# axruff/cuda-flow3d

Measured on AMD Instinct MI355X. Metric: Mvoxels/s full pyramid solve, higher is better.
Workload: dtype f32; 1 GPU; 512^3 synthetic translated-Gaussian float32 pair (BASELINE config 4), full coarse-to-fine pyramid (40 levels x 40 outer x 5 inner, alpha 7.5, median 5^3, Gaussian sigma 2), frames resident in HBM (value = device-resident rate); parallelism=1 GPU

## Files before the change

cuda-flow3d_amd/csrc/f3d_pair8_plan.h:

```cpp
#pragma once

#include <algorithm>
#include <cstdlib>
#include <vector>

#if !defined(__HIPCC__) && !defined(__host__)
#define __host__
#define __device__
#define F3D_PAIR8_PLAN_OWN_QUALIFIERS
#endif

constexpr int kPair8Lanes = 64;

#if defined(__HIP_DEVICE_COMPILE__)
#define PAIR8_UNIFORM(x) __builtin_amdgcn_readfirstlane(x)
#else
#define PAIR8_UNIFORM(x) (x)
#endif

inline int solver_chunk_limit(unsigned long long plane_bytes, int reach)
{
  if (plane_bytes == 0 || plane_bytes > 0x100000000ull || reach < 0) return 0;
  const long long planes = static_cast<long long>(0xffffffffull / plane_bytes) - 8;
  if (planes >= 1) return planes > 0x3fffffff ? 0x3fffffff : static_cast<int>(planes);
// ... 42 lines not shown
  const int n_a = tiles_a * PAIR8_UNIFORM(c.chunks_a), n_b = tiles_b * PAIR8_UNIFORM(c.chunks_b), n_c = tiles_c * PAIR8_UNIFORM(c.chunks_c);
  int cls;
  int item;
  if (xcd_remap) {
    const int per_a = (n_a + 7) / 8, per_b = (n_b + 7) / 8, per_c = (n_c + 7) / 8;
    const int xcd = wg % 8, s = wg / 8;
    cls = s < per_a ? 0 : (s < per_a + per_b ? 1 : 2);
    item = cls == 0 ? xcd * per_a + s : (cls == 1 ? xcd * per_b + (s - per_a) : xcd * per_c + (s - per_a - per_b));
  } else {
    cls = wg < n_a ? 0 : (wg < n_a + n_b ? 1 : 2);
    item = cls == 0 ? wg : (cls == 1 ? wg - n_a : wg - n_a - n_b);
  }
  if (item >= (cls == 0 ? n_a : (cls == 1 ? n_b : n_c))) return false;
  const int tiles = cls == 0 ? tiles_a : (cls == 1 ? tiles_b : tiles_c);
  const int zc = cls == 0 ? zc_a : (cls == 1 ? zc_b : zc_c);
  const int chunk = item / tiles;
  w.tile = item % tiles + (cls == 0 ? 0 : (cls == 1 ? tiles_a : tiles_a + tiles_b));
  w.z0 = m_lo + chunk * zc;
  w.z1 = w.z0 + zc + more < m_hi ? w.z0 + zc + more : m_hi;
  if (fold) {
    const int pair = w.tile / (2 * ntx - 1), k = w.tile % (2 * ntx - 1);
    w.folded = k == ntx - 1;
    w.tx = k < ntx ? k : k - ntx;
    w.ty = k < ntx ? 2 * pair : 2 * pair + 1;
  } else {
    w.folded = false;
    w.tx = w.tile % ntx;
    w.ty = w.tile / ntx;
  }
  return true;
}

__host__ __device__ constexpr int pair8_slot_halo_off(int ns, int nj) { return ns * nj * kPair8Lanes; }
__host__ __device__ constexpr int pair8_slot_floats(int ns, int nj)
{
  return pair8_slot_halo_off(ns, nj) + (ns * 2 * nj + kPair8Lanes - 1) / kPair8Lanes * 4 * kPair8Lanes;
}
struct Pair8XNeighbours {
  int left, right;
};
__host__ __device__ inline Pair8XNeighbours pair8_x_neighbours(int lane, int x0, int width)
{
  const int x = x0 + lane;
  Pair8XNeighbours n = {lane - 1, lane + 1};
  if (x == 0) n.left = n.right;
  if (x == width - 1) n.right = n.left;
  return n;
}
__host__ __device__ inline int pair8_x_neighbour_offset(int elem, int array, int row, int ns, int nj)
{
  const int halo = pair8_slot_halo_off(ns, nj) + (array * 2 * nj + row) * 4;
  if (elem < 0) return halo + 3;
  if (elem >= kPair8Lanes) return halo + nj * 4;
  return (array * nj + row) * kPair8Lanes + elem;
}

struct Pair8Plan {
  int zchunk;
  long cost;
  long wgs = 0;
  Pair8Cut cut = {};
};
inline Pair8Cut pair8_uniform_cut(int tiles, int planes, int zchunk)
{
  return Pair8Cut{0, 0, 0, tiles, (planes + zchunk - 1) / zchunk, zchunk, 0, 0, 0};
}
inline long pair8_per_round(long standard)
{
  const char* e = std::getenv("F3D_PAIR8_ROUND");
  const long v = e ? std::atol(e) : 0;
  return v > 0 ? v : standard;
}
inline int pair8_chunk_steps()
{
  static const int extra = std::getenv("F3D_PAIR8_CHUNK_STEPS") ? std::atoi(std::getenv("F3D_PAIR8_CHUNK_STEPS")) : 7;
  return extra;
}
inline Pair8Plan pair8_plan_two(int width, int rows, int planes, int ty, int zc_limit, long per_round, bool fold, bool two_class)
{
  const long tiles = pair8_tiles_per_chunk((width + kPair8Lanes - 1) / kPair8Lanes, (rows + ty - 1) / ty, fold);
  const int max_chunks = planes > 0 ? planes : 1;
  const int extra = pair8_chunk_steps();
  auto rounds = [&](long wgs) { return (wgs + per_round - 1) / per_round; };
  Pair8Plan p = {std::min(planes, zc_limit), -1};
  for (int nzc = 1; nzc <= max_chunks; ++nzc) {
    const int zc = (planes + nzc - 1) / nzc;
    if (zc > zc_limit) continue;
    const long wgs = tiles * ((planes + zc - 1) / zc);
    const long cost = rounds(wgs) * (zc + extra);
    if (p.cost < 0 || cost < p.cost) {
      p.cost = cost;
      p.zchunk = zc;
      p.wgs = wgs;
    }
  }
  if (p.cost < 0) {
    p.cost = static_cast<long>(rounds(tiles)) * (p.zchunk + extra);
    p.wgs = tiles;
  }
  if (p.zchunk < 1) p.zchunk = 1;
  p.cut = pair8_uniform_cut(static_cast<int>(tiles), planes, p.zchunk);
  if (!two_class || tiles <= per_round || planes < 1 || zc_limit < 1) return p;
  const int a0 = (planes + zc_limit - 1) / zc_limit;
  int zc_a_seen = 0;
  for (int na = a0; na <= a0 + 2 && na <= planes; ++na) {
    const int zc_a = (planes + na - 1) / na;
// ... 126 lines not shown
```

cuda-flow3d_amd/csrc/f3d_solve_pair8.h:

```cpp

enum { PAIR_SS = 0, PAIR_SP = 1, PAIR_PS = 2, PAIR_SSA = 3 };

struct PairArgs {
  const float* in[12];
  float* out[5];
  float hx, hy, hz, alpha;
  float eps_s, eps_d;
  int plain_division;
  int keep_below, keep_above;
  double r4[3], r2[3];
  float d4[3], d2[3];
  float w[3];
  float eps_s2, eps_d2;
  int fdivs_ok, sdivs_ok;
};

inline bool pair_weights_finite(float hx, float hy, float hz, float alpha)
{
  for (float h : {hx, hy, hz}) {
    const float w = alpha / (h * h);
    if (!(w - w == 0.f) || std::signbit(w)) return false;
  }
  return true;
}
// ... 138 lines not shown
    phi = w_phi;
    ksi = w_ksi;
  } else {
    phi = weight_ieee(a_phi);
    ksi = weight_ieee(a_ksi);
  }
}

__device__ __forceinline__ void weights_first_stage1(float (&q)[9], bool with_ksi, float fx, float fy, float fz, float ft, float du,
                                                     float dv_c, float dw, const SolveDivs& dv, float eps_s2, float eps_d2, float& phi,
                                                     float& ksi, bool counts, bool fast_weights)
{
  if (__builtin_expect(dv.ok, 1)) {
#pragma unroll
    for (int c = 0; c < 3; ++c) {
      q[3 * c + 0] = udiv(q[3 * c + 0], dv.x2);
      q[3 * c + 1] = udiv(q[3 * c + 1], dv.y2);
      q[3 * c + 2] = udiv(q[3 * c + 2], dv.z2);
    }
  } else {
#pragma unroll
    for (int c = 0; c < 3; ++c) {
      q[3 * c + 0] = q[3 * c + 0] / dv.x2.d;
      q[3 * c + 1] = q[3 * c + 1] / dv.y2.d;
      q[3 * c + 2] = q[3 * c + 2] / dv.z2.d;
    }
  }
  const float dux = q[0], duy = q[1], duz = q[2], dvx = q[3], dvy = q[4], dvz = q[5], dwx = q[6], dwy = q[7], dwz = q[8];
  const float a_phi = dux * dux + duy * duy + duz * duz + dvx * dvx + dvy * dvy + dvz * dvz + dwx * dwx + dwy * dwy + dwz * dwz + eps_s2;
  float s_phi, s_ksi = 1.f, a_ksi = 1.f, w_ksi = 0.f;
  const float w_phi = weight_fast(a_phi, s_phi);
  bool lane_ok = weight_fast_ok(a_phi, s_phi);
  if (with_ksi) {
    const float J11 = fx * fx, J22 = fy * fy, J33 = fz * fz;
    const float J12 = fx * fy, J13 = fx * fz, J23 = fy * fz;
    const float J14 = fx * ft, J24 = fy * ft, J34 = fz * ft, J44 = ft * ft;
    float s = (J11 * du + J12 * dv_c + J13 * dw + J14) * du + (J12 * du + J22 * dv_c + J23 * dw + J24) * dv_c +
              (J13 * du + J23 * dv_c + J33 * dw + J34) * dw + (J14 * du + J24 * dv_c + J34 * dw + J44);
    s = static_cast<float>(s > 0) * s;
    a_ksi = s + eps_d2;
    w_ksi = weight_fast(a_ksi, s_ksi);
    lane_ok = lane_ok && weight_fast_ok(a_ksi, s_ksi);
  }
  if (__builtin_expect(fast_weights && __builtin_amdgcn_ballot_w64(counts && !lane_ok) == 0, 1)) {
    phi = w_phi;
    ksi = w_ksi;
  } else {
    phi = weight_ieee(a_phi);
    ksi = with_ksi ? weight_ieee(a_ksi) : 0.f;
  }
}


template <int MODE, int TY, int ABL, bool FD, bool YM, bool TIGHT, bool FOLDS = false>
__device__ __forceinline__ void pair8_body(const PairArgs& a, const F3dGeo& g, const Pair8Cut& cut, int ntx, int nty, int xcd_remap)
{
  static_assert(!FOLDS || (!YM && !TIGHT && ABL == 0), "two row bands per tile: z-marching product builds only");
  static_assert(!(YM && FD), "the frame-derivative launchers march along z only");
  static_assert(!TIGHT || (YM && ABL == 0), "a tile without halo rows holds every row of the volume: thin volumes marched along y");
  constexpr bool PS = MODE == PAIR_PS;
  constexpr bool SSM = MODE == PAIR_SS || MODE == PAIR_SSA;
  static_assert((!PS && MODE != PAIR_SSA) || (FD && !YM && !TIGHT && ABL == 0), "k_wpair8: frame-derivative z-marching product builds only");
  constexpr int RH = TIGHT ? 0 : 1;
  const int RDIM = YM ? g.D : g.H;
  const int MDIM = YM ? g.H : g.D;
  const int m_lo = YM ? 0 : g.z_lo, m_hi = YM ? g.H : g.z_hi;
  constexpr int NA = FD ? 12 : 10;
  using L = Pair8Lds<TY, NA, FD, TIGHT, PS>;
  constexpr int NR = L::NR, NJ = L::NJ, NK = L::NK, NJP = L::NJP, NH = L::NH;
  static_assert(TY <= 32, "the column wave holds one halo voxel per lane: 2 x TY <= 64");
  __shared__ __attribute__((aligned(16))) float ring[L::kSlots][L::kSlotFloats];
  __shared__ __attribute__((aligned(16))) float cring[L::kCSlots][L::kCSlotFloats];
  constexpr int SB = FD ? 2 : 0;
  constexpr int NI = PS ? 4 : 3;
  constexpr int IW = kLanes + 2;
  constexpr int IS = (NR * IW + 63) / 64 * 64;
  __shared__ float imgx[2][PS ? NI : 1][PS ? IS : 1];
  __shared__ float img1[2][NI][PS ? 1 : NR][kLanes];
  __shared__ float hc1[2][NI][2][32];
  __shared__ float img3[(ABL & 64) ? 3 : 1][(ABL & 64) ? NR : 1][(ABL & 64) ? kLanes : 1];

  Pair8Wg wg;
  if (!pair8_decode(static_cast<int>(blockIdx.x), cut, ntx, nty, FOLDS, xcd_remap, m_lo, m_hi, (ABL & 64) ? 1 : 0, wg)) return;
  const int tx = wg.tx, ty = wg.ty;
  const bool folded = wg.folded;

  auto tile_body = [&](auto fold_c) __attribute__((always_inline)) {
  constexpr bool FOLD = decltype(fold_c)::value;
  int lane = threadIdx.x;
  const int r = __builtin_amdgcn_readfirstlane(static_cast<int>(threadIdx.y));
  const bool colw = r == NR;
  const bool loader = r == NR + 1;
  const int z0 = wg.z0, z1 = wg.z1;
  const int qs = z0 > 0 ? z0 - 1 : 0;
  const int qe = z1 < MDIM ? z1 : MDIM - 1;
  const int q_end = z1 < MDIM ? qe : qe + 1;
  const int p_last = qe + 1;
  const int x0 = tx * kLanes;
  const int y0 = ty * TY;
  const bool left_face = tx == 0;
  const bool right_face = x0 + kLanes >= g.W;
  const bool tile_at_x_face = __builtin_amdgcn_readfirstlane(static_cast<int>(left_face || right_face)) != 0;
  const bool col_at_x_face = __builtin_amdgcn_readfirstlane(static_cast<int>(left_face || right_face || x0 + kLanes == g.W - 1)) != 0;

  const int st_lo = (a.keep_below && z0 == m_lo) ? z0 - 1 : z0;
  const int st_hi = (a.keep_above && z1 == m_hi) ? z1 + 1 : z1;
  const int zb = qs > 0 ? qs - 1 : 0;
  const unsigned z_stride_b = static_cast<unsigned>(g.Hc) * static_cast<unsigned>(g.pitch) * 4u;
  const unsigned y_stride_b = static_cast<unsigned>(g.pitch) * 4u;
  const unsigned plane_b = YM ? y_stride_b : z_stride_b;
  const unsigned row_b = YM ? z_stride_b : y_stride_b;
  const size_t base_off = YM ? static_cast<size_t>(zb) * static_cast<size_t>(g.pitch) : f3d_row(g, 0, zb);

  if (loader) {
    __builtin_amdgcn_s_setprio(3);
    const float* base[NA];
#pragma unroll
    for (int i = 0; i < NA; ++i) base[i] = (PS && (i == 8 || i == 9)) ? nullptr : uniform_ptr(a.in[i] + base_off);
    const bool bandb = FOLD && (lane & 15) >= 8;
    const int seg = bandb ? (lane & 15) - 8 : (lane & 15);
    unsigned rowb[NK];
    bool rowv[NK];
#pragma unroll
    for (int k = 0; k < NK; ++k) {
      const int j = 4 * k + (lane >> 4);
      rowv[k] = j < NJ;
      const int yrow = f3d_clampi(f3d_mir(y0 + (bandb ? TY : 0) - 2 * RH + (rowv[k] ? j : 0), RDIM), 0, RDIM - 1);
      rowb[k] = static_cast<unsigned>(yrow) * row_b + static_cast<unsigned>(x0 + 4 * seg) * 4u;
    }
    const float* hptr[NH];
    bool hv[NH];
#pragma unroll
// ... 152 lines not shown
        static_cast<int>(static_cast<unsigned>(zz - zb) * plane_b + static_cast<unsigned>(yrow) * row_b)));
  };

  float seedv = static_cast<float>(lane) * 0.01f + 1.f;
  auto fake_raw = [&](PlaneRegs& p) __attribute__((always_inline)) {
    p.f0 = opaque(seedv); p.f1 = opaque(seedv); p.u = opaque(seedv); p.v = opaque(seedv); p.w = opaque(seedv);
    p.su = opaque(seedv); p.dv = opaque(seedv); p.dw = opaque(seedv); p.phi = opaque(seedv); p.ksi = opaque(seedv);
    p.fz = opaque(seedv); p.ft = opaque(seedv);
  };
  auto row_raw = [&](PlaneRegs& p, const float* slot, int j, bool with_ksi, const float* cs = nullptr) __attribute__((always_inline)) {
    if (ABL & 8) return fake_raw(p);
    const float* d = slot + j * kLanes + lane;
    constexpr int st = NJP * kLanes;
    if (!FD) {
      p.f0 = d[F0 * st];
      p.f1 = d[F1 * st];
    }
    p.u = d[(U - SB) * st]; p.v = d[(V - SB) * st]; p.w = d[(Wf - SB) * st];
    p.su = d[(DU - SB) * st]; p.dv = d[(DV - SB) * st]; p.dw = d[(DW - SB) * st]; p.phi = d[(PHI - SB) * st];
    if (!FD && with_ksi) p.ksi = d[9 * st];
    if (FD && !with_ksi) p.f0 = p.f1 = 0.f;
    if (FD && with_ksi) {
      const float* c = cs + (j - 1) * kLanes + lane;
      constexpr int ct = L::NRC * kLanes;
      p.f0 = c[0 * ct]; p.f1 = c[1 * ct]; p.ksi = c[2 * ct]; p.fz = c[3 * ct]; p.ft = c[4 * ct];
    }
  };
  auto halo_raw = [&](PlaneRegs& p, const float* slot, int s, int j, int e, bool with_ksi, const float* cs = nullptr) __attribute__((always_inline)) {
    if (ABL & 8) return fake_raw(p);
    const float* d = slot + L::kHaloOff + (s * NJ + j) * 4 + e;
    constexpr int st = 2 * NJ * 4;
    if (!FD) {
      p.f0 = d[F0 * st];
      p.f1 = d[F1 * st];
    }
    p.u = d[(U - SB) * st]; p.v = d[(V - SB) * st]; p.w = d[(Wf - SB) * st];
    p.su = d[(DU - SB) * st]; p.dv = d[(DV - SB) * st]; p.dw = d[(DW - SB) * st]; p.phi = d[(PHI - SB) * st];
    if (!FD && with_ksi) p.ksi = d[9 * st];
    if (FD && !with_ksi) p.f0 = p.f1 = 0.f;
    if (FD && with_ksi) {
      const float* c = cs + L::kCHaloOff + (s * TY + (j - 2)) * 4 + e;
      constexpr int ct = 2 * TY * 4;
      p.f0 = c[0 * ct]; p.f1 = c[1 * ct]; p.ksi = c[2 * ct]; p.fz = c[3 * ct]; p.ft = c[4 * ct];
    }
  };

  S3 hM = {0.f, 0.f, 0.f}, hC = {0.f, 0.f, 0.f};
  float hC_dv = 0.f, hC_dw = 0.f;
  Carry kC = {};
  Carry kC2 = {};
  CarryP pC = {};

  Face6 nYm = {}, nYp = {}, nX = {};
  S3 nDy = {0.f, 0.f, 0.f}, nXr = {0.f, 0.f, 0.f};
  Face6 nIn = {};
  S3 nInr = {0.f, 0.f, 0.f};
  auto fetch_neighbours = [&](auto colw_c, const float* S) __attribute__((always_inline)) {
    constexpr bool CW = decltype(colw_c)::value;
    PlaneRegs T0, T1, T2;
    if constexpr (CW) {
      PlaneRegs T;
      const float* d = S + jc * kLanes + (side ? (FOLD ? 32 : kLanes - 1) : 0);
      constexpr int st = NJP * kLanes;
      if (ABL & 8) {
        fake_raw(T);
      } else {
        if (!FD) {
          T.f0 = d[F0 * st];
          T.f1 = d[F1 * st];
        } else {
          T.f0 = T.f1 = 0.f;
        }
        T.u = d[(U - SB) * st]; T.v = d[(V - SB) * st]; T.w = d[(Wf - SB) * st];
        T.su = d[(DU - SB) * st]; T.dv = d[(DV - SB) * st]; T.dw = d[(DW - SB) * st]; T.phi = d[(PHI - SB) * st];
      }
      nInr = {T.u, T.v, T.w};
      plane_finish(T);
      nIn = plane_face(T);
    }
    if constexpr (CW) {
      halo_raw(T0, S, side, jc_m, e_near, false);
      halo_raw(T1, S, side, jc_p, e_near, false);
      halo_raw(T2, S, side, jc, e_far, false);
    } else {
      row_raw(T0, S, jr_m, false);
      row_raw(T1, S, jr_p, false);
      halo_raw(T2, S, side, jr, e_near, false);
    }
    if (MODE == PAIR_SP) {
      nDy = {T1.u - T0.u, T1.v - T0.v, T1.w - T0.w};
      nXr = {T2.u, T2.v, T2.w};
    }
    plane_finish(T0);
    plane_finish(T1);
    plane_finish(T2);
    nYm = plane_face(T0);
    nYp = plane_face(T1);
    nX = plane_face(T2);
  };

  auto step = [&](auto colw_c, auto slot_c, PlaneRegs& M, PlaneRegs& C, PlaneRegs& P, int q) __attribute__((always_inline)) {
    constexpr bool CW = decltype(colw_c)::value;
    constexpr int SLOT = decltype(slot_c)::value;
    if constexpr (TY > 8 || TIGHT) lane = fresh_lane();
    const int band = FOLD ? lane >> 5 : 0;
    if (!(ABL & 8)) __syncthreads();
    if (ABL & 4) return;
    const float* Sp = &ring[SLOT][0];
    const float* Cp = &cring[FD ? ((q + 1 - qs) & 1) : 0][0];
    const bool do1 = q <= qe;
    const int b = q & 1;

    float r_du = 0.f, r_dv = 0.f, r_dw = 0.f;
    Carry kN;
    CarryP pN;
    {
      Face6 xm, xp;
      const Face6 ym = nYm, yp = nYp;
      S3 rxm = {}, rxp = {};
      int vx, vy;
      if constexpr (CW) {
        halo_raw(P, Sp, side, jc, e_near, true, Cp);
        plane_finish(P);
        const S3 router = nXr;
        const Face6 outer = nX;
        const S3 rinner = nInr;
        const Face6 inner = nIn;
#pragma unroll
        for (int i = 0; i < kNL; ++i) {
          xm.v[i] = !FOLD && side ? inner.v[i] : outer.v[i];
          xp.v[i] = !FOLD && side ? outer.v[i] : inner.v[i];
        }
        rxm = !FOLD && side ? rinner : router;
        rxp = !FOLD && side ? router : rinner;
        vx = cx;
        vy = cy;
        if (cx == g.W - 1) {
          xp = xm;
          rxp = rxm;
        }
      } else {
        row_raw(P, Sp, jr, true, Cp);
        plane_finish(P);
        const S3 rx = nXr;
        const Face6 xf = nX;
        const Face6 cf = plane_face(C);
#pragma unroll
        for (int i = 0; i < kNL; ++i) {
          xm.v[i] = left_or(cf.v[i], xf.v[i]);
          xp.v[i] = lane_right_or(cf.v[i], xf.v[i]);
        }
        if (MODE == PAIR_SP) {
          rxm = {left_or(C.u, rx.u), left_or(C.v, rx.v), left_or(C.w, rx.w)};
          rxp = {lane_right_or(C.u, rx.u), lane_right_or(C.v, rx.v), lane_right_or(C.w, rx.w)};
        }
        vx = x;
        vy = band ? y + TY : y;
        if (tile_at_x_face) {
          if (x == 0) {
            xm = xp;
            rxm = rxp;
          }
          if (x == g.W - 1) {
            xp = xm;
            rxp = rxm;
          }
        }
      }
      const Face6 cfc = plane_face(C);
      if (ABL & 2) {
        kN = Carry{};
        r_du = xm.v[0] + xp.v[1] + ym.v[2] + yp.v[3] + M.su + P.sv + C.ksi + rxm.u + nDy.v;
        r_dv = xm.v[4] + xp.v[5] + ym.v[0] + yp.v[1] + M.f0 + P.f1 + C.u + rxp.w + nDy.u;
        r_dw = xm.v[2] + xp.v[3] + ym.v[4] + yp.v[5] + M.phi + P.phi + C.dv + C.dw + C.v + C.w;
        kN.J12 = r_du; kN.d1 = r_dv; kN.pw[0] = r_dw;
      } else
      {
        const Face6 fM = plane_face(M), fP = plane_face(P);
        const bool row_p = vy < RDIM - 1, row_m = vy > 0, mar_p = q < MDIM - 1, mar_m = q > 0;
        constexpr bool FDA = FD || (ABL & 16) != 0;
        sweep_stage1<FDA, true>(xm, xp, YM ? fM : ym, YM ? fP : yp, YM ? ym : fM, YM ? yp : fP, cfc.v, C.u, C.v, C.w, C.dv, C.dw,
                                C.ksi, a.hx, a.hy, a.hz, fdivs, a.alpha, vx < g.W - 1, vx > 0, YM ? mar_p : row_p, YM ? mar_m : row_m,
                                YM ? row_p : mar_p, YM ? row_m : mar_m, r_du, r_dv, r_dw, kN, C.f0, C.f1, FD ? C.fz : C.phi,
                                FD ? C.ft : C.ksi, CW ? col_at_x_face : tile_at_x_face, a.w[0], a.w[1], a.w[2]);
      }
      pN.fx = kN.fx; pN.fy = kN.fy; pN.fz = kN.fz; pN.ft = kN.ft;
      {
        const S3 dRow = nDy, dMar = {P.u - M.u, P.v - M.v, P.w - M.w};
        const S3 dY = YM ? dMar : dRow, dZ = YM ? dRow : dMar;
        pN.D[0] = rxp.u - rxm.u; pN.D[1] = dY.u; pN.D[2] = dZ.u;
        pN.D[3] = rxp.v - rxm.v; pN.D[4] = dY.v; pN.D[5] = dZ.v;
        pN.D[6] = rxp.w - rxm.w; pN.D[7] = dY.w; pN.D[8] = dZ.w;
      }
    }
    const S3 sN = SSM ? S3{C.u + r_du, C.v + r_dv, C.w + r_dw} : S3{r_du, r_dv, r_dw};
    if (do1 && !(ABL & 8)) {
      if constexpr (CW) {
        if (cactive) {
          hc1[b][0][side][crow] = sN.u;
          hc1[b][1][side][crow] = sN.v;
          hc1[b][2][side][crow] = sN.w;
        }
      } else {
        img1[b][0][r][lane] = sN.u;
        img1[b][1][r][lane] = sN.v;
        img1[b][2][r][lane] = sN.w;
      }
    }
    if (MODE == PAIR_SP && do1 && owner && q >= st_lo && q < st_hi) {
      const unsigned off = xb + rowoff(yy, q);
      gst(obase[0], off, r_du);
      gst(obase[1], off, r_dv);
      gst(obase[2], off, r_dw);
    }

    const int t = q - 1;
    const bool do2 = !CW && core && t >= z0;
    float o0 = 0.f, o1 = 0.f, o2 = 0.f;
    if (do2) {
      const int pb = t & 1;
      S3 ym, yp, xm, xp, zm, zp;
      float eu, ev, ew;
      if (ABL & 8) {
        ym.u = opaque(seedv); ym.v = opaque(seedv); ym.w = opaque(seedv);
        yp.u = opaque(seedv); yp.v = opaque(seedv); yp.w = opaque(seedv);
        eu = opaque(seedv); ev = opaque(seedv); ew = opaque(seedv);
      } else {
        const int im = band ? r_ymb : r_ym, ip = band ? r_ypb : r_yp;
        ym.u = img1[pb][0][im][lane]; ym.v = img1[pb][1][im][lane]; ym.w = img1[pb][2][im][lane];
        yp.u = img1[pb][0][ip][lane]; yp.v = img1[pb][1][ip][lane]; yp.w = img1[pb][2][ip][lane];
        eu = hc1[pb][0][side][r - RH]; ev = hc1[pb][1][side][r - RH]; ew = hc1[pb][2][side][r - RH];
      }
      xm.u = left_or(hC.u, eu); xm.v = left_or(hC.v, ev); xm.w = left_or(hC.w, ew);
      xp.u = lane_right_or(hC.u, eu); xp.v = lane_right_or(hC.v, ev); xp.w = lane_right_or(hC.w, ew);
      zm = hM;
      zp = sN;
      if (tile_at_x_face) {
        if (x == 0) xm = xp;
        if (x == g.W - 1) xp = xm;
      }
      if (t == 0) zm = zp;
      if (t == MDIM - 1) zp = zm;
      if (ABL & 2) {
        o0 = xm.u + xp.v + ym.w + kC.J12;
        o1 = yp.u + zm.v + zp.w + kC.d1;
        o2 = xm.w + yp.v + zp.u + kC.pw[0] + hC_dv + hC_dw;
      } else if (SSM)
      {
        sweep_stage2(kC, xm, xp, YM ? zm : ym, YM ? zp : yp, YM ? ym : zm, YM ? yp : zp, hC_dv, hC_dw, o0, o1, o2);
        if constexpr (MODE == PAIR_SSA) {
          o0 = kC.U + o0;
          o1 = kC.V + o1;
          o2 = kC.W + o2;
        }
      } else
        phi_ksi_stage2(pC, xm, xp, YM ? zm : ym, YM ? zp : yp, YM ? ym : zm, YM ? yp : zp, hC.u, hC.v, hC.w, sdivs, a.eps_s2,
                       a.eps_d2, o0, o1, owner, a.plain_division == 0);
    }
    if constexpr ((ABL & 64) != 0) {
      if (do2) {
        img3[0][r][lane] = o0; img3[1][r][lane] = o1; img3[2][r][lane] = o2;
        S3 ym, yp, xm, xp;
        ym.u = img3[0][r_ym][lane]; ym.v = img3[1][r_ym][lane]; ym.w = img3[2][r_ym][lane];
        yp.u = img3[0][r_yp][lane]; yp.v = img3[1][r_yp][lane]; yp.w = img3[2][r_yp][lane];
        const float eu = hc1[b][0][side][r - 1], ev = hc1[b][1][side][r - 1], ew = hc1[b][2][side][r - 1];
        xm.u = lane_left_or(o0, eu); xm.v = lane_left_or(o1, ev); xm.w = lane_left_or(o2, ew);
        xp.u = lane_right_or(o0, eu); xp.v = lane_right_or(o1, ev); xp.w = lane_right_or(o2, ew);
        const S3 zm = hM, zp = {o0, o1, o2};
        float p0, p1, p2;
        sweep_stage2(kC2, xm, xp, ym, yp, zm, zp, o1, o2, p0, p1, p2);
        o0 = p0; o1 = p1; o2 = p2;
      }
      kC2 = kC;
    }
    asm volatile("" ::"v"(o0), "v"(o1), "v"(o2), "v"(sN.u), "v"(sN.v), "v"(sN.w));
    hM = hC;
    hC = sN;
    hC_dv = r_dv;
    hC_dw = r_dw;
    kC = kN;
    pC = pN;
    if (do2 && owner) {
      const unsigned off = xb + rowoff(yy, t);
      if (SSM) {
        gst(obase[0], off, o0);
        gst(obase[1], off, o1);
        gst(obase[2], off, o2);
      } else {
        gst(obase[3], off, o0);
        gst(obase[4], off, o1);
      }
    }
    fetch_neighbours(colw_c, Sp);
  };


  auto row_raw_ps = [&](PlaneRegs& p, const float* slot, int j, bool centre, const float* cs) __attribute__((always_inline)) {
    const float* d = slot + j * kLanes + lane;
    constexpr int st = NJP * kLanes;
    p.u = d[0 * st]; p.v = d[1 * st]; p.w = d[2 * st];
    p.su = d[3 * st]; p.dv = d[4 * st]; p.dw = d[5 * st];
    p.ksi = p.su;
    if (centre) {
      const float* c = cs + (j - 2) * kLanes + lane;
      constexpr int ct = L::NRC * kLanes;
      p.f0 = c[0 * ct]; p.f1 = c[1 * ct]; p.fz = c[2 * ct]; p.ft = c[3 * ct];
    }
  };
  auto halo_raw_ps = [&](PlaneRegs& p, const float* slot, int s, int j, int e) __attribute__((always_inline)) {
    const float* d = slot + L::kHaloOff + (s * NJ + j) * 4 + e;
    constexpr int st = 2 * NJ * 4;
    p.u = d[0 * st]; p.v = d[1 * st]; p.w = d[2 * st];
    p.su = d[3 * st]; p.dv = d[4 * st]; p.dw = d[5 * st];
    p.ksi = p.su;
  };
  S3 nXd = {0.f, 0.f, 0.f}, nInd = {0.f, 0.f, 0.f};
  unsigned xaL[6] = {}, xaR[6] = {};
  S3 nDx = {0.f, 0.f, 0.f};
  float phM = 0.f, phC = 0.f, ksC = 0.f;
  auto fetch_ps = [&](auto colw_c, const float* S) __attribute__((always_inline)) {
    constexpr bool CW = decltype(colw_c)::value;
    PlaneRegs T0, T1, T2;
    if constexpr (CW) {
      PlaneRegs T;
      const float* d = S + jc * kLanes + (side ? (FOLD ? 32 : kLanes - 1) : 0);
      constexpr int st = NJP * kLanes;
      T.u = d[0 * st]; T.v = d[1 * st]; T.w = d[2 * st]; T.su = d[3 * st]; T.dv = d[4 * st]; T.dw = d[5 * st];
      nInr = {T.u, T.v, T.w};
      nInd = {T.su, T.dv, T.dw};
      halo_raw_ps(T0, S, side, jc_m, e_near);
      halo_raw_ps(T1, S, side, jc_p, e_near);
      halo_raw_ps(T2, S, side, jc, e_far);
    } else {
      row_raw_ps(T0, S, jr_m, false, nullptr);
      row_raw_ps(T1, S, jr_p, false, nullptr);
      if constexpr (FOLD) {
        halo_raw_ps(T2, S, side, jr, e_near);
      } else {
        float xl[6], xr[6];
#pragma unroll
        for (int i = 0; i < 6; ++i) {
          xl[i] = *reinterpret_cast<const float*>(reinterpret_cast<const char*>(S) + xaL[i]);
          xr[i] = *reinterpret_cast<const float*>(reinterpret_cast<const char*>(S) + xaR[i]);
        }
        nDx = {((xr[0] - xl[0]) + xr[3]) - xl[3], ((xr[1] - xl[1]) + xr[4]) - xl[4], ((xr[2] - xl[2]) + xr[5]) - xl[5]};
      }
    }
    nDy = {((T1.u - T0.u) + T1.su) - T0.su, ((T1.v - T0.v) + T1.dv) - T0.dv, ((T1.w - T0.w) + T1.dw) - T0.dw};
    if constexpr (CW || FOLD) {
      nXr = {T2.u, T2.v, T2.w};
      nXd = {T2.su, T2.dv, T2.dw};
    }
  };
  auto step_ps = [&](auto colw_c, auto slot_c, PlaneRegs& M, PlaneRegs& C, PlaneRegs& P, int q) __attribute__((always_inline)) {
    constexpr bool CW = decltype(colw_c)::value;
    constexpr int SLOT = decltype(slot_c)::value;
    if constexpr (TY > 8) lane = fresh_lane();
    const int band = FOLD ? lane >> 5 : 0;
    __syncthreads();
    const float* Sp = &ring[SLOT][0];
    const float* Cp = &cring[(q + 1 - qs) & 1][0];
    const bool do1 = q <= qe;
    const int b = q & 1;
    auto ix = [&](int buf, int comp, int row, int col) __attribute__((always_inline)) -> float& { return imgx[buf][comp][row * IW + col]; };
    if constexpr (CW) halo_raw_ps(P, Sp, side, jc, e_near);
    else row_raw_ps(P, Sp, jr, core, Cp);
    plane_finish(P);

    S3 rxm, rxp, dxm, dxp;
    int vx, vy;
    if constexpr (CW) {
      rxm = !FOLD && side ? nInr : nXr;
      rxp = !FOLD && side ? nXr : nInr;
      dxm = !FOLD && side ? nInd : nXd;
      dxp = !FOLD && side ? nXd : nInd;
      vx = cx;
      vy = cy;
      if (cx == g.W - 1) {
        rxp = rxm;
        dxp = dxm;
      }
    } else if constexpr (FOLD) {
      rxm = {left_or(C.u, nXr.u), left_or(C.v, nXr.v), left_or(C.w, nXr.w)};
      rxp = {lane_right_or(C.u, nXr.u), lane_right_or(C.v, nXr.v), lane_right_or(C.w, nXr.w)};
      dxm = {left_or(C.ksi, nXd.u), left_or(C.dv, nXd.v), left_or(C.dw, nXd.w)};
      dxp = {lane_right_or(C.ksi, nXd.u), lane_right_or(C.dv, nXd.v), lane_right_or(C.dw, nXd.w)};
      vx = x;
      vy = band ? y + TY : y;
      if (tile_at_x_face) {
        if (x == 0) {
          rxm = rxp;
          dxm = dxp;
        }
        if (x == g.W - 1) {
          rxp = rxm;
          dxp = dxm;
        }
      }
    } else {
      vx = x;
      vy = y;
    }
    float nq[9] = {0.f, nDy.u, ((P.u - M.u) + P.ksi) - M.ksi, 0.f, nDy.v, ((P.v - M.v) + P.dv) - M.dv,
                   0.f, nDy.w, ((P.w - M.w) + P.dw) - M.dw};
    if constexpr (CW || FOLD) {
      nq[0] = ((rxp.u - rxm.u) + dxp.u) - dxm.u;
      nq[3] = ((rxp.v - rxm.v) + dxp.v) - dxm.v;
      nq[6] = ((rxp.w - rxm.w) + dxp.w) - dxm.w;
    } else {
      nq[0] = nDx.u;
      nq[3] = nDx.v;
      nq[6] = nDx.w;
    }
    const bool counts = do1 && vx >= 0 && vx < g.W && vy >= 0 && vy < RDIM && (!CW || cactive);
    float phi_q = 0.f, ksi_q = 0.f;
    weights_first_stage1(nq, !CW && core, C.f0, C.f1, C.fz, C.ft, C.ksi, C.dv, C.dw, sdivs, a.eps_s2, a.eps_d2, phi_q, ksi_q, counts,
                         a.plain_division == 0);
    constexpr int IX = FOLD ? 0 : 1;
    if (do1) {
      if constexpr (CW) {
        if (cactive) {
          if constexpr (FOLD) {
            hc1[b][0][side][crow] = C.su;
            hc1[b][1][side][crow] = C.sv;
            hc1[b][2][side][crow] = C.sw;
            hc1[b][3][side][crow] = phi_q;
          } else {
            const int pad = side ? kLanes + 1 : 0;
            ix(b, 0, RH + crow, pad) = C.su;
            ix(b, 1, RH + crow, pad) = C.sv;
            ix(b, 2, RH + crow, pad) = C.sw;
            ix(b, 3, RH + crow, pad) = phi_q;
          }
        }
      } else {
        ix(b, 0, r, lane + IX) = C.su;
        ix(b, 1, r, lane + IX) = C.sv;
        ix(b, 2, r, lane + IX) = C.sw;
        ix(b, 3, r, lane + IX) = phi_q;
      }
    }
    if (!CW && do1 && owner && q >= z0 && q < z1) {
      const unsigned off = xb + rowoff(yy, q);
      gst(obase[3], off, phi_q);
      gst(obase[4], off, ksi_q);
    }

    const int t = q - 1;
    const bool do2 = !CW && core && t >= z0;
    if (do2) {
      float o0, o1, o2;
      const int pb = t & 1;
      const int im = band ? r_ymb : r_ym, ip = band ? r_ypb : r_yp;
      Face6 ym = {}, yp = {}, xm = {}, xp = {}, zm = {}, zp = {}, cf = {};
      const int li = lane + IX;
      ym.v[LSU] = ix(pb, 0, im, li); ym.v[LSV] = ix(pb, 1, im, li); ym.v[LSW] = ix(pb, 2, im, li); ym.v[LPHI] = ix(pb, 3, im, li);
      yp.v[LSU] = ix(pb, 0, ip, li); yp.v[LSV] = ix(pb, 1, ip, li); yp.v[LSW] = ix(pb, 2, ip, li); yp.v[LPHI] = ix(pb, 3, ip, li);
      cf.v[LSU] = M.su; cf.v[LSV] = M.sv; cf.v[LSW] = M.sw; cf.v[LPHI] = phC;
      if constexpr (FOLD) {
        const float eu = hc1[pb][0][side][r - RH], ev = hc1[pb][1][side][r - RH], ew = hc1[pb][2][side][r - RH], ep = hc1[pb][3][side][r - RH];
        xm.v[LSU] = left_or(M.su, eu); xm.v[LSV] = left_or(M.sv, ev); xm.v[LSW] = left_or(M.sw, ew); xm.v[LPHI] = left_or(phC, ep);
        xp.v[LSU] = lane_right_or(M.su, eu); xp.v[LSV] = lane_right_or(M.sv, ev); xp.v[LSW] = lane_right_or(M.sw, ew);
        xp.v[LPHI] = lane_right_or(phC, ep);
      } else {
        xm.v[LSU] = ix(pb, 0, r, lane); xm.v[LSV] = ix(pb, 1, r, lane); xm.v[LSW] = ix(pb, 2, r, lane); xm.v[LPHI] = ix(pb, 3, r, lane);
        xp.v[LSU] = ix(pb, 0, r, lane + 2); xp.v[LSV] = ix(pb, 1, r, lane + 2); xp.v[LSW] = ix(pb, 2, r, lane + 2);
        xp.v[LPHI] = ix(pb, 3, r, lane + 2);
      }
      zm.v[LSU] = hM.u; zm.v[LSV] = hM.v; zm.v[LSW] = hM.w; zm.v[LPHI] = phM;
      zp.v[LSU] = C.su; zp.v[LSV] = C.sv; zp.v[LSW] = C.sw; zp.v[LPHI] = phi_q;
      if (tile_at_x_face) {
        if (x == 0) xm = xp;
        if (x == g.W - 1) xp = xm;
      }
      if (t == 0) zm = zp;
      if (t == MDIM - 1) zp = zm;
      Carry kU;
      sweep_stage1<true, true>(xm, xp, ym, yp, zm, zp, cf.v, M.u, M.v, M.w, M.dv, M.dw, ksC, a.hx, a.hy, a.hz, fdivs, a.alpha, vx < g.W - 1,
                               vx > 0, vy < RDIM - 1, vy > 0, t < MDIM - 1, t > 0, o0, o1, o2, kU, M.f0, M.f1, M.fz, M.ft, tile_at_x_face,
                               a.w[0], a.w[1], a.w[2]);
      asm volatile("" ::"v"(o0), "v"(o1), "v"(o2), "v"(phi_q));
      if (owner) {
        const unsigned off = xb + rowoff(yy, t);
        gst(obase[0], off, o0);
        gst(obase[1], off, o1);
        gst(obase[2], off, o2);
      }
    }
    hM = {M.su, M.sv, M.sw};
    phM = phC;
    phC = phi_q;
    ksC = ksi_q;
    fetch_ps(colw_c, Sp);
  };

  __syncthreads();
  PlaneRegs A = {}, B = {}, Cc = {};
  const float* Sm = &ring[0][0];
  const float* S0 = &ring[1][0];
  using Slot0 = std::integral_constant<int, 0>;
  using Slot1 = std::integral_constant<int, 1>;
  using Slot2 = std::integral_constant<int, 2>;
  auto march = [&](auto colw_c) __attribute__((always_inline)) {
    constexpr bool CW = decltype(colw_c)::value;
    if constexpr (PS) {
      if constexpr (CW) {
        halo_raw_ps(A, Sm, side, jc, e_near);
        halo_raw_ps(B, S0, side, jc, e_near);
      } else {
        row_raw_ps(A, Sm, jr, false, nullptr);
        row_raw_ps(B, S0, jr, core, &cring[0][0]);
      }
    } else if constexpr (CW) {
      halo_raw(A, Sm, side, jc, e_near, false);
      halo_raw(B, S0, side, jc, e_near, true, &cring[0][0]);
    } else {
      row_raw(A, Sm, jr, false);
      row_raw(B, S0, jr, true, &cring[0][0]);
    }
    plane_finish(A);
    plane_finish(B);
    int q = qs;
    if constexpr (PS) {
      if constexpr (!CW && !FOLD) {
        static_assert(pair8_slot_halo_off(L::NS, NJ) == L::kHaloOff && pair8_slot_floats(L::NS, NJ) == L::kSlotFloats && L::NS == 6 && NJP == NJ,
                      "pair8_x_neighbour_offset describes this slot");
        const Pair8XNeighbours xn = pair8_x_neighbours(lane, x0, g.W);
#pragma unroll
        for (int i = 0; i < 6; ++i) {
          xaL[i] = 4u * static_cast<unsigned>(pair8_x_neighbour_offset(xn.left, i, jr, L::NS, NJ));
          xaR[i] = 4u * static_cast<unsigned>(pair8_x_neighbour_offset(xn.right, i, jr, L::NS, NJ));
          asm volatile("" : "+v"(xaL[i]));
          asm volatile("" : "+v"(xaR[i]));
        }
      }
      fetch_ps(colw_c, S0);
      for (; q + 2 <= q_end; q += 3) {
        step_ps(colw_c, Slot2{}, A, B, Cc, q);
        step_ps(colw_c, Slot0{}, B, Cc, A, q + 1);
        step_ps(colw_c, Slot1{}, Cc, A, B, q + 2);
      }
      if (q <= q_end) step_ps(colw_c, Slot2{}, A, B, Cc, q);
      if (q + 1 <= q_end) step_ps(colw_c, Slot0{}, B, Cc, A, q + 1);
    } else {
      fetch_neighbours(colw_c, S0);
      for (; q + 2 <= q_end; q += 3) {
        step(colw_c, Slot2{}, A, B, Cc, q);
        step(colw_c, Slot0{}, B, Cc, A, q + 1);
        step(colw_c, Slot1{}, Cc, A, B, q + 2);
      }
      if (q <= q_end) step(colw_c, Slot2{}, A, B, Cc, q);
      if (q + 1 <= q_end) step(colw_c, Slot0{}, B, Cc, A, q + 1);
    }
  };
  if (colw) march(std::true_type{});
  else march(std::false_type{});
  asm volatile("s_waitcnt vmcnt(0)" ::: "memory");
  };
  if constexpr (FOLDS) {
    if (__builtin_amdgcn_readfirstlane(static_cast<int>(folded))) return tile_body(std::true_type{});
  }
  tile_body(std::false_type{});
}

template <int MODE, int TY, int ABL = 0, bool FD = false, bool YM = false, bool FOLDS = false>
__global__ __launch_bounds__(kLanes*(TY + 4)) void k_pair8(PairArgs a, F3dGeo g, Pair8Cut cut, int ntx, int nty, int xcd_remap)
{
  pair8_body<MODE, TY, ABL, FD, YM, false, FOLDS>(a, g, cut, ntx, nty, xcd_remap);
}
template <int MODE, int TY, bool FOLDS>
__global__ __launch_bounds__(kLanes*(TY + 4)) void k_wpair8(PairArgs a, F3dGeo g, Pair8Cut cut, int ntx, int nty, int xcd_remap)
{
  pair8_body<MODE, TY, 0, true, false, false, FOLDS>(a, g, cut, ntx, nty, xcd_remap);
}
template <int MODE, int TY>
__global__ __launch_bounds__(kLanes*(TY + 2)) __attribute__((amdgpu_waves_per_eu(4))) void k_pair8t(PairArgs a, F3dGeo g, Pair8Cut cut, int ntx,
                                                                                                   int nty, int xcd_remap)
{
  pair8_body<MODE, TY, 0, false, true, true>(a, g, cut, ntx, nty, xcd_remap);
}

inline Pair8Plan pair8_plan_launch_kept(int width, int rows, int planes, int ty, int zc_limit, long per_round, bool fold)
{
  struct Key {
    int width, rows, planes, ty, zc_limit, fold, plan;
    long per_round;
    bool operator==(const Key& o) const
    {
      return width == o.width && rows == o.rows && planes == o.planes && ty == o.ty && zc_limit == o.zc_limit && fold == o.fold &&
             plan == o.plan && per_round == o.per_round;
    }
  };
  thread_local Key keys[3] = {};
  thread_local Pair8Plan plans[3] = {};
  const char* pe = std::getenv("F3D_PAIR8_PLAN");
  const Key key = {width, rows, planes, ty, zc_limit, fold ? 1 : 0, pe ? pe[0] : 0, per_round};
  const int slot = ty <= 4 ? 0 : (ty <= 8 ? 1 : 2);
// ... 104 lines not shown
```

Before: 80.60 Mvoxels/s.

## Read x-neighbours of both sweeps from LDS via precomputed addresses, extend to folded tiles

For the z-marching SS/SSA builds, the second sweep's intermediate field is now staged in a padded per-row LDS image (imgx) instead of row images plus column-halo buffers. X-neighbours come from that padded image rather than from cross-lane shuffles with halo selection. Stage 1 can also read left and right neighbours directly from the ring slot using per-lane precomputed byte offsets. Folded two-band tiles get matching address helpers, so the weights-first PS path also uses LDS loads instead of shuffles. The aim is to replace DPP/permute lane shifts and their edge-select logic with plain LDS reads, at the cost of more LDS traffic, extra address registers and a larger shared footprint.

After: 81.26 Mvoxels/s, median of 6. About the same (+0.8%).

```diff
diff --git a/cuda-flow3d_amd/csrc/f3d_pair8_plan.h b/cuda-flow3d_amd/csrc/f3d_pair8_plan.h
--- a/cuda-flow3d_amd/csrc/f3d_pair8_plan.h
+++ b/cuda-flow3d_amd/csrc/f3d_pair8_plan.h
@@ -118,6 +118,23 @@
   const int halo = pair8_slot_halo_off(ns, nj) + (array * 2 * nj + row) * 4;
   if (elem < 0) return halo + 3;
   if (elem >= kPair8Lanes) return halo + nj * 4;
+  return (array * nj + row) * kPair8Lanes + elem;
+}
+
+__host__ __device__ inline Pair8XNeighbours pair8_x_neighbours_folded(int lane, int x0, int width)
+{
+  const int band = lane / (kPair8Lanes / 2), c = lane % (kPair8Lanes / 2);
+  const int x = x0 + c;
+  Pair8XNeighbours n = {c == 0 ? -1 - band : lane - 1, lane + 1};
+  if (x == 0) n.left = n.right;
+  if (x >= width - 1) n.right = n.left;
+  return n;
+}
+__host__ __device__ inline int pair8_x_neighbour_offset_folded(int elem, int array, int row, int ns, int nj)
+{
+  const int halo = pair8_slot_halo_off(ns, nj) + (array * 2 * nj + row) * 4;
+  if (elem == -1) return halo + 3;
+  if (elem == -2) return halo + nj * 4 + 3;
   return (array * nj + row) * kPair8Lanes + elem;
 }
 
diff --git a/cuda-flow3d_amd/csrc/f3d_solve_pair8.h b/cuda-flow3d_amd/csrc/f3d_solve_pair8.h
--- a/cuda-flow3d_amd/csrc/f3d_solve_pair8.h
+++ b/cuda-flow3d_amd/csrc/f3d_solve_pair8.h
@@ -214,6 +214,18 @@
 }
 
 
+constexpr bool pair8_stage1_from_ring(int mode, int ty, bool fd, bool fold)
+{
+  if (ty == 4 && (fold || !fd)) return false;
+  if (ty == 12 && fold && !fd) return false;
+  return true;
+}
+constexpr bool pair8_two_sweeps_from_lds(int mode, int ty, bool fd, bool folds)
+{
+  return !(fd && ty == 12 && (folds || mode == PAIR_SSA));
+}
+constexpr bool kWeightsFirstFoldFromLds = true;
+
 template <int MODE, int TY, int ABL, bool FD, bool YM, bool TIGHT, bool FOLDS = false>
 __device__ __forceinline__ void pair8_body(const PairArgs& a, const F3dGeo& g, const Pair8Cut& cut, int ntx, int nty, int xcd_remap)
 {
@@ -235,11 +247,13 @@
   __shared__ __attribute__((aligned(16))) float cring[L::kCSlots][L::kCSlotFloats];
   constexpr int SB = FD ? 2 : 0;
   constexpr int NI = PS ? 4 : 3;
+  constexpr bool XI = SSM && !YM && !TIGHT && ABL == 0 && pair8_two_sweeps_from_lds(MODE, TY, FD, FOLDS);
+  constexpr bool PX = PS || XI;
   constexpr int IW = kLanes + 2;
   constexpr int IS = (NR * IW + 63) / 64 * 64;
-  __shared__ float imgx[2][PS ? NI : 1][PS ? IS : 1];
-  __shared__ float img1[2][NI][PS ? 1 : NR][kLanes];
-  __shared__ float hc1[2][NI][2][32];
+  __shared__ float imgx[2][PX ? NI : 1][PX ? IS : 1];
+  __shared__ float img1[2][NI][PX ? 1 : NR][kLanes];
+  __shared__ float hc1[2][NI][2][(XI || (PS && kWeightsFirstFoldFromLds)) ? 1 : 32];
   __shared__ float img3[(ABL & 64) ? 3 : 1][(ABL & 64) ? NR : 1][(ABL & 64) ? kLanes : 1];
 
   Pair8Wg wg;
@@ -498,6 +512,10 @@
   CarryP pC = {};
 
   Face6 nYm = {}, nYp = {}, nX = {};
+  constexpr bool XB = XI && pair8_stage1_from_ring(MODE, TY, FD, FOLD);
+  constexpr int NX = FD ? 7 : 9;
+  Face6 nXm = {}, nXp = {};
+  unsigned xaL[9] = {}, xaR[9] = {};
   S3 nDy = {0.f, 0.f, 0.f}, nXr = {0.f, 0.f, 0.f};
   Face6 nIn = {};
   S3 nInr = {0.f, 0.f, 0.f};
@@ -531,18 +549,39 @@
     } else {
       row_raw(T0, S, jr_m, false);
       row_raw(T1, S, jr_p, false);
-      halo_raw(T2, S, side, jr, e_near, false);
-    }
-    if (MODE == PAIR_SP) {
-      nDy = {T1.u - T0.u, T1.v - T0.v, T1.w - T0.w};
-      nXr = {T2.u, T2.v, T2.w};
-    }
-    plane_finish(T0);
-    plane_finish(T1);
-    plane_finish(T2);
-    nYm = plane_face(T0);
-    nYp = plane_face(T1);
-    nX = plane_face(T2);
+      if constexpr (!XB) halo_raw(T2, S, side, jr, e_near, false);
+    }
+    if constexpr (!CW && XB) {
+      PlaneRegs TL, TR;
+      auto at = [&](unsigned off) __attribute__((always_inline)) {
+        return *reinterpret_cast<const float*>(reinterpret_cast<const char*>(S) + off);
+      };
+      TL.f0 = FD ? 0.f : at(xaL[F0]); TL.f1 = FD ? 0.f : at(xaL[F1]);
+      TR.f0 = FD ? 0.f : at(xaR[F0]); TR.f1 = FD ? 0.f : at(xaR[F1]);
+      TL.u = at(xaL[U - SB]); TL.v = at(xaL[V - SB]); TL.w = at(xaL[Wf - SB]);
+      TL.su = at(xaL[DU - SB]); TL.dv = at(xaL[DV - SB]); TL.dw = at(xaL[DW - SB]); TL.phi = at(xaL[PHI - SB]);
+      TR.u = at(xaR[U - SB]); TR.v = at(xaR[V - SB]); TR.w = at(xaR[Wf - SB]);
+      TR.su = at(xaR[DU - SB]); TR.dv = at(xaR[DV - SB]); TR.dw = at(xaR[DW - SB]); TR.phi = at(xaR[PHI - SB]);
+      plane_finish(T0);
+      plane_finish(T1);
+      plane_finish(TL);
+      plane_finish(TR);
+      nYm = plane_face(T0);
+      nYp = plane_face(T1);
+      nXm = plane_face(TL);
+      nXp = plane_face(TR);
+    } else {
+      if (MODE == PAIR_SP) {
+        nDy = {T1.u - T0.u, T1.v - T0.v, T1.w - T0.w};
+        nXr = {T2.u, T2.v, T2.w};
+      }
+      plane_finish(T0);
+      plane_finish(T1);
+      plane_finish(T2);
+      nYm = plane_face(T0);
+      nYp = plane_face(T1);
+      nX = plane_face(T2);
+    }
   };
 
   auto step = [&](auto colw_c, auto slot_c, PlaneRegs& M, PlaneRegs& C, PlaneRegs& P, int q) __attribute__((always_inline)) {
@@ -588,28 +627,33 @@
       } else {
         row_raw(P, Sp, jr, true, Cp);
         plane_finish(P);
-        const S3 rx = nXr;
-        const Face6 xf = nX;
-        const Face6 cf = plane_face(C);
-#pragma unroll
-        for (int i = 0; i < kNL; ++i) {
-          xm.v[i] = left_or(cf.v[i], xf.v[i]);
-          xp.v[i] = lane_right_or(cf.v[i], xf.v[i]);
-        }
-        if (MODE == PAIR_SP) {
-          rxm = {left_or(C.u, rx.u), left_or(C.v, rx.v), left_or(C.w, rx.w)};
-          rxp = {lane_right_or(C.u, rx.u), lane_right_or(C.v, rx.v), lane_right_or(C.w, rx.w)};
-        }
         vx = x;
         vy = band ? y + TY : y;
-        if (tile_at_x_face) {
-          if (x == 0) {
-            xm = xp;
-            rxm = rxp;
+        if constexpr (XB) {
+          xm = nXm;
+          xp = nXp;
+        } else {
+          const S3 rx = nXr;
+          const Face6 xf = nX;
+          const Face6 cf = plane_face(C);
+#pragma unroll
+          for (int i = 0; i < kNL; ++i) {
+            xm.v[i] = left_or(cf.v[i], xf.v[i]);
+            xp.v[i] = lane_right_or(cf.v[i], xf.v[i]);
           }
-          if (x == g.W - 1) {
-            xp = xm;
-            rxp = rxm;
+          if (MODE == PAIR_SP) {
+            rxm = {left_or(C.u, rx.u), left_or(C.v, rx.v), left_or(C.w, rx.w)};
+            rxp = {lane_right_or(C.u, rx.u), lane_right_or(C.v, rx.v), lane_right_or(C.w, rx.w)};
+          }
+          if (tile_at_x_face) {
+            if (x == 0) {
+              xm = xp;
+              rxm = rxp;
+            }
+            if (x == g.W - 1) {
+              xp = xm;
+              rxp = rxm;
+            }
           }
         }
       }
@@ -640,7 +684,23 @@
       }
     }
     const S3 sN = SSM ? S3{C.u + r_du, C.v + r_dv, C.w + r_dw} : S3{r_du, r_dv, r_dw};
-    if (do1 && !(ABL & 8)) {
+    auto ix = [&](int buf, int comp, int row, int col) __attribute__((always_inline)) -> float& { return imgx[buf][comp][row * IW + col]; };
+    if constexpr (XI) {
+      if (do1) {
+        if constexpr (CW) {
+          if (cactive) {
+            const int pad = side ? kLanes + 1 : 0;
+            ix(b, 0, RH + crow, pad) = sN.u;
+            ix(b, 1, RH + crow, pad) = sN.v;
+            ix(b, 2, RH + crow, pad) = sN.w;
+          }
+        } else {
+          ix(b, 0, r, lane + 1) = sN.u;
+          ix(b, 1, r, lane + 1) = sN.v;
+          ix(b, 2, r, lane + 1) = sN.w;
+        }
+      }
+    } else if (do1 && !(ABL & 8)) {
       if constexpr (CW) {
         if (cactive) {
           hc1[b][0][side][crow] = sN.u;
@@ -671,14 +731,23 @@
         ym.u = opaque(seedv); ym.v = opaque(seedv); ym.w = opaque(seedv);
         yp.u = opaque(seedv); yp.v = opaque(seedv); yp.w = opaque(seedv);
         eu = opaque(seedv); ev = opaque(seedv); ew = opaque(seedv);
+      } else if constexpr (XI) {
+        const int im = band ? r_ymb : r_ym, ip = band ? r_ypb : r_yp;
+        const int li = lane + 1, lm = FOLD && lane == 32 ? kLanes + 1 : lane;
+        ym.u = ix(pb, 0, im, li); ym.v = ix(pb, 1, im, li); ym.w = ix(pb, 2, im, li);
+        yp.u = ix(pb, 0, ip, li); yp.v = ix(pb, 1, ip, li); yp.w = ix(pb, 2, ip, li);
+        xm.u = ix(pb, 0, r, lm); xm.v = ix(pb, 1, r, lm); xm.w = ix(pb, 2, r, lm);
+        xp.u = ix(pb, 0, r, lane + 2); xp.v = ix(pb, 1, r, lane + 2); xp.w = ix(pb, 2, r, lane + 2);
       } else {
         const int im = band ? r_ymb : r_ym, ip = band ? r_ypb : r_yp;
         ym.u = img1[pb][0][im][lane]; ym.v = img1[pb][1][im][lane]; ym.w = img1[pb][2][im][lane];
         yp.u = img1[pb][0][ip][lane]; yp.v = img1[pb][1][ip][lane]; yp.w = img1[pb][2][ip][lane];
         eu = hc1[pb][0][side][r - RH]; ev = hc1[pb][1][side][r - RH]; ew = hc1[pb][2][side][r - RH];
       }
-      xm.u = left_or(hC.u, eu); xm.v = left_or(hC.v, ev); xm.w = left_or(hC.w, ew);
-      xp.u = lane_right_or(hC.u, eu); xp.v = lane_right_or(hC.v, ev); xp.w = lane_right_or(hC.w, ew);
+      if constexpr (!XI) {
+        xm.u = left_or(hC.u, eu); xm.v = left_or(hC.v, ev); xm.w = left_or(hC.w, ew);
+        xp.u = lane_right_or(hC.u, eu); xp.v = lane_right_or(hC.v, ev); xp.w = lane_right_or(hC.w, ew);
+      }
       zm = hM;
       zp = sN;
       if (tile_at_x_face) {
@@ -761,7 +830,7 @@
     p.ksi = p.su;
   };
   S3 nXd = {0.f, 0.f, 0.f}, nInd = {0.f, 0.f, 0.f};
-  unsigned xaL[6] = {}, xaR[6] = {};
+  constexpr bool SHF = FOLD && !kWeightsFirstFoldFromLds;
   S3 nDx = {0.f, 0.f, 0.f};
   float phM = 0.f, phC = 0.f, ksC = 0.f;
   auto fetch_ps = [&](auto colw_c, const float* S) __attribute__((always_inline)) {
@@ -780,7 +849,7 @@
     } else {
       row_raw_ps(T0, S, jr_m, false, nullptr);
       row_raw_ps(T1, S, jr_p, false, nullptr);
-      if constexpr (FOLD) {
+      if constexpr (SHF) {
         halo_raw_ps(T2, S, side, jr, e_near);
       } else {
         float xl[6], xr[6];
@@ -793,7 +862,7 @@
       }
     }
     nDy = {((T1.u - T0.u) + T1.su) - T0.su, ((T1.v - T0.v) + T1.dv) - T0.dv, ((T1.w - T0.w) + T1.dw) - T0.dw};
-    if constexpr (CW || FOLD) {
+    if constexpr (CW || SHF) {
       nXr = {T2.u, T2.v, T2.w};
       nXd = {T2.su, T2.dv, T2.dw};
     }
@@ -826,7 +895,7 @@
         rxp = rxm;
         dxp = dxm;
       }
-    } else if constexpr (FOLD) {
+    } else if constexpr (SHF) {
       rxm = {left_or(C.u, nXr.u), left_or(C.v, nXr.v), left_or(C.w, nXr.w)};
       rxp = {lane_right_or(C.u, nXr.u), lane_right_or(C.v, nXr.v), lane_right_or(C.w, nXr.w)};
       dxm = {left_or(C.ksi, nXd.u), left_or(C.dv, nXd.v), left_or(C.dw, nXd.w)};
@@ -845,11 +914,11 @@
       }
     } else {
       vx = x;
-      vy = y;
+      vy = band ? y + TY : y;
     }
     float nq[9] = {0.f, nDy.u, ((P.u - M.u) + P.ksi) - M.ksi, 0.f, nDy.v, ((P.v - M.v) + P.dv) - M.dv,
                    0.f, nDy.w, ((P.w - M.w) + P.dw) - M.dw};
-    if constexpr (CW || FOLD) {
+    if constexpr (CW || SHF) {
       nq[0] = ((rxp.u - rxm.u) + dxp.u) - dxm.u;
       nq[3] = ((rxp.v - rxm.v) + dxp.v) - dxm.v;
       nq[6] = ((rxp.w - rxm.w) + dxp.w) - dxm.w;
@@ -862,11 +931,11 @@
     float phi_q = 0.f, ksi_q = 0.f;
     weights_first_stage1(nq, !CW && core, C.f0, C.f1, C.fz, C.ft, C.ksi, C.dv, C.dw, sdivs, a.eps_s2, a.eps_d2, phi_q, ksi_q, counts,
                          a.plain_division == 0);
-    constexpr int IX = FOLD ? 0 : 1;
+    constexpr int IX = SHF ? 0 : 1;
     if (do1) {
       if constexpr (CW) {
         if (cactive) {
-          if constexpr (FOLD) {
+          if constexpr (SHF) {
             hc1[b][0][side][crow] = C.su;
             hc1[b][1][side][crow] = C.sv;
             hc1[b][2][side][crow] = C.sw;
@@ -903,13 +972,14 @@
       ym.v[LSU] = ix(pb, 0, im, li); ym.v[LSV] = ix(pb, 1, im, li); ym.v[LSW] = ix(pb, 2, im, li); ym.v[LPHI] = ix(pb, 3, im, li);
       yp.v[LSU] = ix(pb, 0, ip, li); yp.v[LSV] = ix(pb, 1, ip, li); yp.v[LSW] = ix(pb, 2, ip, li); yp.v[LPHI] = ix(pb, 3, ip, li);
       cf.v[LSU] = M.su; cf.v[LSV] = M.sv; cf.v[LSW] = M.sw; cf.v[LPHI] = phC;
-      if constexpr (FOLD) {
+      if constexpr (SHF) {
         const float eu = hc1[pb][0][side][r - RH], ev = hc1[pb][1][side][r - RH], ew = hc1[pb][2][side][r - RH], ep = hc1[pb][3][side][r - RH];
         xm.v[LSU] = left_or(M.su, eu); xm.v[LSV] = left_or(M.sv, ev); xm.v[LSW] = left_or(M.sw, ew); xm.v[LPHI] = left_or(phC, ep);
         xp.v[LSU] = lane_right_or(M.su, eu); xp.v[LSV] = lane_right_or(M.sv, ev); xp.v[LSW] = lane_right_or(M.sw, ew);
         xp.v[LPHI] = lane_right_or(phC, ep);
       } else {
-        xm.v[LSU] = ix(pb, 0, r, lane); xm.v[LSV] = ix(pb, 1, r, lane); xm.v[LSW] = ix(pb, 2, r, lane); xm.v[LPHI] = ix(pb, 3, r, lane);
+        const int lm = FOLD && lane == 32 ? kLanes + 1 : lane;
+        xm.v[LSU] = ix(pb, 0, r, lm); xm.v[LSV] = ix(pb, 1, r, lm); xm.v[LSW] = ix(pb, 2, r, lm); xm.v[LPHI] = ix(pb, 3, r, lm);
         xp.v[LSU] = ix(pb, 0, r, lane + 2); xp.v[LSV] = ix(pb, 1, r, lane + 2); xp.v[LSW] = ix(pb, 2, r, lane + 2);
         xp.v[LPHI] = ix(pb, 3, r, lane + 2);
       }
@@ -968,14 +1038,16 @@
     plane_finish(B);
     int q = qs;
     if constexpr (PS) {
-      if constexpr (!CW && !FOLD) {
+      if constexpr (!CW && !SHF) {
         static_assert(pair8_slot_halo_off(L::NS, NJ) == L::kHaloOff && pair8_slot_floats(L::NS, NJ) == L::kSlotFloats && L::NS == 6 && NJP == NJ,
                       "pair8_x_neighbour_offset describes this slot");
-        const Pair8XNeighbours xn = pair8_x_neighbours(lane, x0, g.W);
+        const Pair8XNeighbours xn = FOLD ? pair8_x_neighbours_folded(lane, x0, g.W) : pair8_x_neighbours(lane, x0, g.W);
 #pragma unroll
         for (int i = 0; i < 6; ++i) {
-          xaL[i] = 4u * static_cast<unsigned>(pair8_x_neighbour_offset(xn.left, i, jr, L::NS, NJ));
-          xaR[i] = 4u * static_cast<unsigned>(pair8_x_neighbour_offset(xn.right, i, jr, L::NS, NJ));
+          xaL[i] = 4u * static_cast<unsigned>(FOLD ? pair8_x_neighbour_offset_folded(xn.left, i, jr, L::NS, NJ)
+                                                   : pair8_x_neighbour_offset(xn.left, i, jr, L::NS, NJ));
+          xaR[i] = 4u * static_cast<unsigned>(FOLD ? pair8_x_neighbour_offset_folded(xn.right, i, jr, L::NS, NJ)
+                                                   : pair8_x_neighbour_offset(xn.right, i, jr, L::NS, NJ));
           asm volatile("" : "+v"(xaL[i]));
           asm volatile("" : "+v"(xaR[i]));
         }
@@ -989,6 +1061,20 @@
       if (q <= q_end) step_ps(colw_c, Slot2{}, A, B, Cc, q);
       if (q + 1 <= q_end) step_ps(colw_c, Slot0{}, B, Cc, A, q + 1);
     } else {
+      if constexpr (!CW && XB) {
+        static_assert(pair8_slot_halo_off(L::NS, NJ) == L::kHaloOff && pair8_slot_floats(L::NS, NJ) == L::kSlotFloats && NX <= L::NS && NJP == NJ,
+                      "pair8_x_neighbour_offset describes this slot");
+        const Pair8XNeighbours xn = FOLD ? pair8_x_neighbours_folded(lane, x0, g.W) : pair8_x_neighbours(lane, x0, g.W);
+#pragma unroll
+        for (int i = 0; i < NX; ++i) {
+          xaL[i] = 4u * static_cast<unsigned>(FOLD ? pair8_x_neighbour_offset_folded(xn.left, i, jr, L::NS, NJ)
+                                                   : pair8_x_neighbour_offset(xn.left, i, jr, L::NS, NJ));
+          xaR[i] = 4u * static_cast<unsigned>(FOLD ? pair8_x_neighbour_offset_folded(xn.right, i, jr, L::NS, NJ)
+                                                   : pair8_x_neighbour_offset(xn.right, i, jr, L::NS, NJ));
+          asm volatile("" : "+v"(xaL[i]));
+          asm volatile("" : "+v"(xaR[i]));
+        }
+      }
       fetch_neighbours(colw_c, S0);
       for (; q + 2 <= q_end; q += 3) {
         step(colw_c, Slot2{}, A, B, Cc, q);
```
